# DJjjjhao/FIRA-ICSE

Hardware: AMD Instinct MI355X
Metric: training commits/sec (FIRA default config) (higher is better)
Workload: dtype f32; 1 GPU; BASELINE configs[1]: FIRA training step (fwd+bwd+Adam, dropout 0.1/0.2), batch 32 commits/GPU, fp32, 650-node graphs (mean nnz 1066/graph), vocab 24650; global_batch=32, parallelism=dp1

## Files before the change

### fira_icse_amd/csrc/engine.hip

```cpp
#include "engine.h"
#include <hip/hip_ext.h>
#include "epilogue.h"
#include <stdlib.h>
#include <map>
#include <mutex>

namespace fira {

static int64_t shadow_wbt_elems(const Layout& L);

struct Arena {
    char* base;
    size_t used = 0;
    explicit Arena(void* b) : base((char*)b) {}
    template <typename T>
    T* get(size_t n) {
        size_t bytes = (n * sizeof(T) + 255) / 256 * 256;
        T* p = base ? (T*)(base + used) : nullptr;
        used += bytes;
        return p;
    }
    float* f(size_t n) { return get<float>(n); }
};

// ... 257 lines not shown
        return gemm_bf16_ex(s, tA, tB, M, N, K, A, lda, B, ldb, C, ldc, bias, flags, splitk, colsum, c_rows, relu_mask);
    }
    return gemm_f32_ex(s, tA, tB, M, N, K, A, lda, B, ldb, C, ldc, bias, flags, splitk, colsum, c_rows, relu_mask);
}

static inline int linear(hipStream_t s, int M, int N, int K, const float* X, int ldx, const float* W, const float* b,
                         float* Y, int ldy, int flags = 0) {
    return gemm_any(s, 0, 1, M, N, K, X, ldx, W, K, Y, ldy, b, flags, 0, nullptr);
}
static inline int linear_ln(hipStream_t s, int M, int K, const float* X, int ldx, const float* W, const float* b,
                            const float* res, const float* gamma, const float* beta, float* sum, float* y, float* stats,
                            float p_drop, uint64_t seed, uint32_t st, const int32_t* y_rows = nullptr,
                            const float* r1_row = nullptr, const float* r1_col = nullptr,
                            const int32_t* slot2 = nullptr, float* y2 = nullptr, int n2 = 0, const int32_t* rows2 = nullptr,
                            uint32_t idx0 = 0) {
    bool fused = false;
    int rc = 0;
    if (g_dtype != 0 && idx0 == 0 && g_lanes == 1) {
        const uint16_t* wb;
        int ldw;
        fused = shadow_of(W, false, &wb, &ldw) && ldw == K &&
                linear_ln_bf16_try(s, M, K, X, ldx, wb, ldw, b, res, gamma, beta, sum, y, stats, p_drop, seed, st, y_rows, r1_row,
                                   r1_col, &rc);
    }
    if (fused) {
        TRY(rc);
        if (y2 && n2 > 0) TRY(rows_move(s, 0, n2, FIRA_D, y2, y, rows2, nullptr));
        return 0;
    }
    TRY(linear(s, M, FIRA_D, K, X, ldx, W, b, sum, FIRA_D));
    return add_layernorm_fwd(s, M, sum, res, gamma, beta, y, stats, p_drop, seed, st, y_rows, r1_row, r1_col, slot2, y2, idx0);
}
static inline bool linear_presum(hipStream_t s, int M, int K, const float* X, int ldx, const float* W, const float* b,
                                 const float* res, float* sum, float p_drop, uint64_t seed, uint32_t st, int* rc,
                                 uint32_t idx0 = 0) {
    if (g_dtype != 0 || !gemm_tile32_takes(1, M, FIRA_D, K, X, ldx, W, K)) return false;
    EpiRes er;
    er.res = res; er.ldr = FIRA_D; er.p = p_drop; er.inv_keep = p_drop > 0.f ? 1.0f / (1.0f - p_drop) : 1.0f;
    er.seed = seed; er.site = st; er.idx0 = idx0;
    ProfScope prof(s, PROF_GEMM, 2.0 * M * FIRA_D * (double)K, 4.0 * ((double)M * K + (double)FIRA_D * K + 2.0 * M * FIRA_D));
    return gemm_tile32_try(s, 1, M, FIRA_D, K, X, ldx, W, K, sum, FIRA_D, b, 0, rc, nullptr, nullptr, nullptr, &er);
}
static inline int linear_dgrad(hipStream_t s, int M, int N, int K, const float* dY, int lddy, const float* W, float* dX,
                               int lddx, bool accum) {
    return gemm_any(s, 0, 0, M, K, N, dY, lddy, W, K, dX, lddx, nullptr, accum ? FIRA_GEMM_ACCUM : 0, 0, nullptr);
}
struct SideStream {
    hipStream_t stream = nullptr;
    hipStream_t aux = nullptr;
    hipStream_t lane = nullptr;
    std::vector<hipEvent_t> events;
    size_t next = 0;
    bool enabled = true;
    int init() {
        if (stream) return 0;
        const char* off = getenv("FIRA_NO_WGRAD_OVERLAP");
        enabled = !(off && off[0] == '1');
        int least = 0, greatest = 0;
        if (hipDeviceGetStreamPriorityRange(&least, &greatest) != hipSuccess) least = greatest = 0;
        hipError_t e = hipStreamCreateWithPriority(&stream, hipStreamNonBlocking, least);
        if (e != hipSuccess) return set_err("hipStreamCreate: %s", hipGetErrorString(e));
        gemm_set_pad_stream(stream);
        e = hipStreamCreateWithPriority(&aux, hipStreamNonBlocking, greatest);
        if (e != hipSuccess) return set_err("hipStreamCreateWithPriority: %s", hipGetErrorString(e));
        events.resize(512);
        for (auto& ev : events) {
            e = hipEventCreateWithFlags(&ev, hipEventDisableTiming);
            if (e != hipSuccess) return set_err("hipEventCreate: %s", hipGetErrorString(e));
        }
        return 0;
    }
    hipEvent_t ev() { hipEvent_t e = events[next]; next = (next + 1) % events.size(); return e; }
};
static SideStream& side() { static thread_local SideStream s; return s; }

static int side_fork(hipStream_t main_s) {
    SideStream& sd = side();
    hipEvent_t e = sd.ev();
    if (hipEventRecord(e, main_s) != hipSuccess || hipStreamWaitEvent(sd.stream, e, 0) != hipSuccess)
        return set_err("side stream fork failed");
    return 0;
}
struct WaitProbe {
    bool on = false, init = false;
    struct Rec { int line; hipEvent_t a, b; };
    std::vector<Rec> recs;
    std::vector<hipEvent_t> pool;
    int calls = 0;
    bool enabled() {
        if (!init) { const char* e = getenv("FIRA_WAIT_PROBE"); on = e && e[0] == '1'; init = true; }
        return on;
    }
    hipEvent_t ev() {
        if (!pool.empty()) { hipEvent_t e = pool.back(); pool.pop_back(); return e; }
        hipEvent_t e = nullptr;
        (void)hipEventCreate(&e);
        return e;
    }
    void report() {
        (void)hipDeviceSynchronize();
        std::vector<std::pair<int, std::pair<double, int>>> acc;
        for (auto& r : recs) {
            float ms = 0.f;
            if (hipEventElapsedTime(&ms, r.a, r.b) != hipSuccess) ms = 0.f;
            bool found = false;
            for (auto& q : acc) if (q.first == r.line) { q.second.first += ms; q.second.second++; found = true; }
            if (!found) acc.push_back({r.line, {ms, 1}});
            pool.push_back(r.a); pool.push_back(r.b);
        }
        recs.clear();
// ... 186 lines not shown
static inline void note_graph_density(const fira_batch* b) {
    g_dense_graphs = b->n_nodes > 0 && (double)b->nnz > GCN_FUSED_MAX_DEG * (double)b->n_nodes;
}


enum Site { SITE_GATE = 0, SITE_COMB_OUT = 1, SITE_GCN = 2, SITE_SELF = 3, SITE_CROSS = 4, SITE_FFN = 5 };
static inline uint32_t site(int layer, int kind) { return (uint32_t)(layer * 8 + kind + 1); }

struct ClipStep {
    const fira_adam_opts* adam;
    float max_norm;
    fira_clip_state* state;
    void* scratch;
};
struct Ctx {
    hipStream_t s;
    const Layout* L;
    const fira_batch* bt;
    const float* P;
    float* G;
    Plan* pl;
    float p_drop, p_gcn;
    uint64_t seed;
    int R = 0;
    const int32_t* rows = nullptr;
    int Td = 0;
    const int32_t* dec_off = nullptr;
    const int32_t* row_bt = nullptr;
    const int32_t* rows_dense = nullptr;
    bool deferred = false;
    bool kv_ragged = false;
    bool serial = false;
    float* loss_sum = nullptr;
    int32_t* n_tok = nullptr;
    hipEvent_t ev_kv[16] = {};
    int kv_waited = 0;
    hipEvent_t ev_src = nullptr;
    hipEvent_t ev_zero = nullptr;
    const fira_adam_opts* adam = nullptr;
    float* Pw = nullptr;
    bool dp_begin = false;
    bool wout_planes = false;
    bool kv_planes = false;
    int32_t* row_step = nullptr;
    fira_adam_opts rows_ad{};
    bool adam_a_only = false;
    hipEvent_t ev_early = nullptr;
    const float* count = nullptr;
    const ClipStep* clip = nullptr;
    const ShadowTable* shadow_tab = nullptr;
    hipEvent_t ev_shadow = nullptr;
    int n_lanes = 1;
    struct Lane { hipStream_t s; int b0, nb, r0, nr; } lanes[2] = {};
};
typedef Ctx::Lane Lane;

static AdamRowsTables adam_rows_tables(const Layout& L, float* params, const fira_adam_opts& ad, int32_t* row_step) {
    AdamRowsTables tb;
    tb.p = params; tb.m = ad.m; tb.v = ad.v;
    tb.off[0] = L.dec_emb; tb.off[1] = L.emb;
    tb.rows[0] = tb.rows[1] = L.d.vocab;
    tb.last = row_step;
    return tb;
}

static int decoder_lanes(Ctx& c) {
    constexpr int DEC_LANES_MIN_ROWS = 768;
    static const int forced = [] { const char* e = getenv("FIRA_DEC_LANES"); return e ? (atoi(e) >= 2 ? 2 : 1) : 0; }();
    const int want = forced ? forced : (c.Td >= DEC_LANES_MIN_ROWS ? 2 : 1);
    c.n_lanes = g_lanes = 1;
    c.lanes[0] = Lane{c.s, 0, c.pl->B, 0, c.Td};
    const fira_batch& bt = *c.bt;
    if (want < 2 || !c.dec_off || !bt.dec_off_host || bt.B < 2 || !side_on() || c.serial || !c.kv_ragged) return 0;
    SideStream& sd = side();
    if (!sd.lane) {
        if (hipStreamCreateWithFlags(&sd.lane, hipStreamNonBlocking) != hipSuccess) return set_err("lane stream: create failed");
    }
    int bm = 1, best = 1 << 30;
    for (int b = 1; b < bt.B; ++b) {
        const int d = abs(2 * bt.dec_off_host[b] - c.Td);
        if (d < best) { best = d; bm = b; }
    }
    const int rm = bt.dec_off_host[bm];
    if (rm <= 0 || rm >= c.Td || bt.dec_off_host[bt.B] != c.Td) return 0;
    c.n_lanes = g_lanes = 2;
    c.lanes[0] = Lane{c.s, 0, bm, 0, rm};
    c.lanes[1] = Lane{sd.lane, bm, bt.B - bm, rm, c.Td - rm};
    return 0;
}
static int lanes_fork(Ctx& c) {
    for (int k = 1; k < c.n_lanes; ++k) {
        hipEvent_t e = side().ev();
        if (hipEventRecord(e, c.s) != hipSuccess || hipStreamWaitEvent(c.lanes[k].s, e, 0) != hipSuccess) return set_err("lane fork failed");
    }
    return 0;
}
static int lanes_join(Ctx& c) {
    for (int k = 1; k < c.n_lanes; ++k) {
        hipEvent_t e = side().ev();
        if (hipEventRecord(e, c.lanes[k].s) != hipSuccess || hipStreamWaitEvent(c.s, e, 0) != hipSuccess) return set_err("lane join failed");
    }
    return 0;
}
static int lanes_fork_to(Ctx& c, hipStream_t target) {
    for (int k = 0; k < c.n_lanes; ++k) {
        hipEvent_t e = side().ev();
        if (hipEventRecord(e, c.lanes[k].s) != hipSuccess || hipStreamWaitEvent(target, e, 0) != hipSuccess) return set_err("lane -> side stream fork failed");
    }
    return 0;
}

static inline bool fold_one_launch(int nl) { return nl <= 10; }
static inline bool comb_x3_on(int nl) { return nl <= 8; }
static inline bool gcn_x3_on(int nl) { return gcn_fused_on() && fold_one_launch(nl); }
static inline bool kv_x3_on(int nl) { return nl * 2 <= 24; }

static int adam_rows_prefetch(Ctx& c, hipStream_t st) {
    const fira_batch& bt = *c.bt;
    const Plan& p = *c.pl;
    const fira_adam_opts& ad = c.rows_ad;
    AdamRowsLists ls{};
    auto add = [&](const int32_t* ids, int n, int table) {
        if (!ids || n <= 0) return;
        const int k = ls.n_lists++;
        ls.ids[k] = ids; ls.table[k] = table;
        ls.end[k] = (k ? ls.end[k - 1] : 0) + n;
    };
    add(bt.tar, p.B * p.T, 0);
    return adam_rows_catchup(st, adam_rows_tables(*c.L, const_cast<float*>(c.P), ad, c.row_step), &ls, ad.lr, ad.beta1, ad.beta2, ad.eps,
                             ad.step - 1);
}

static int encoder_forward(Ctx& c, bool defer_memory_proj) {
    Plan& p = *c.pl;
    const Layout& L = *c.L;
    const fira_batch& bt = *c.bt;
    hipStream_t s = c.s;
    const int D = FIRA_D, Nc = bt.n_nodes, Cc = bt.n_code, Mc = bt.n_mem, KV = p.nl * 2 * D;
    hipEvent_t ev_fold0 = nullptr, ev_fold = nullptr, ev_comb = nullptr;
    bool fold_waited = false;
    {
        const bool ax = side_on() && !c.serial;
        hipStream_t fs = ax ? side().aux : s;
        if (ax) TRY(aux_fork(s));
        TransposeTable tt;
        for (int l = 0; l < p.nl && tt.n + 3 <= 24; ++l) {
            const EncLayer& w = L.enc[l];
            float* dst = p.WcT + (size_t)l * 3 * D * D;
            tt.src[tt.n] = c.P + w.wqk; tt.dst[tt.n++] = dst;
            tt.src[tt.n] = c.P + w.wqk + (size_t)D * D; tt.dst[tt.n++] = dst + (size_t)D * D;
            tt.src[tt.n] = c.P + w.wo; tt.dst[tt.n++] = dst + (size_t)2 * D * D;
        }
        TRY(transpose256_table(fs, tt));
        if (comb_x3_on(p.nl)) {
            const float* src[48];
            uint16_t* dst[48];
            int n = 0;
            for (int l = 0; l < p.nl; ++l) {
                const EncLayer& w = L.enc[l];
                const float* st[3] = {c.P + w.wqk, c.P + w.wqk + (size_t)D * D, c.P + w.wo};
                for (int j = 0; j < 3; ++j) {
                    src[n] = st[j]; dst[n++] = p.WcX + ((size_t)l * 3 + j) * 3 * D * D;
                    if (c.G) { src[n] = p.WcT + ((size_t)l * 3 + j) * D * D; dst[n++] = p.WcTX + ((size_t)l * 3 + j) * 3 * D * D; }
                }
            }
            TRY(gcn_split_planes(fs, n, src, dst));
        }
        const bool fold_one = fold_one_launch(p.nl);
        if (ax && !(fold_one && (!g_Wb || gcn_fused_on()))) TRY(side_mark(&ev_comb));
        if (fold_one) {
            const float *fW2[16], *fW1[16], *fb1[16];
            for (int l = 0; l < p.nl; ++l) { fW2[l] = c.P + L.enc[l].fc2w; fW1[l] = c.P + L.enc[l].fc1w; fb1[l] = c.P + L.enc[l].fc1b; }
            TRY(gcn_fold_weights(fs, p.nl, fW2, fW1, fb1, p.W21, gcn_fused_on() ? p.W21t : nullptr, p.c21));
            if (gcn_x3_on(p.nl)) {
                const float* src[24];
                uint16_t* dst[24];
                int n = 0;
                for (int l = 0; l < p.nl; ++l) {
                    src[n] = p.W21 + (size_t)l * D * D; dst[n++] = p.W21x + (size_t)l * 3 * D * D;
                    if (c.G) { src[n] = p.W21t + (size_t)l * D * D; dst[n++] = p.W21tx + (size_t)l * 3 * D * D; }
                }
                TRY(gcn_split_planes(fs, n, src, dst));
            }
            if (ax && (!g_Wb || gcn_fused_on())) TRY(side_mark(&ev_fold0));
        } else
        for (int l = 0; l < p.nl; ++l) {
            const EncLayer& w = L.enc[l];
            TRY(gemm_f32_ex(fs, 0, 0, D, D, D, c.P + w.fc2w, D, c.P + w.fc1w, D, p.W21 + (size_t)l * D * D, D, nullptr, 0, 0, nullptr));
            TRY(gemm_f32_ex(fs, 0, 1, D, 1, D, c.P + w.fc2w, D, c.P + w.fc1b, D, p.c21 + (size_t)l * D, 1, nullptr, 0, 0, nullptr));
            if (l == 0 && gcn_fused_on()) TRY(transpose256(fs, 1, p.W21, p.W21t));
            if (ax && l == 0 && !g_Wb && p.nl > 1) TRY(side_mark(&ev_fold0));
        }
        if (g_Wb) {
            ShadowTable t21;
            for (int l = 0; l < p.nl && l < SHADOW_MAX; ++l) {
                t21.e[l] = ShadowEntry{(int64_t)l * D * D, D, D, D, (int64_t)l * D * D};
                t21.tile_start[l + 1] = t21.tile_start[l] + cdiv(D, 64) * cdiv(D, 64);
                t21.n = l + 1;
            }
            TRY(weight_shadows(fs, t21, p.W21, p.w21b, p.w21bt));
            g_W21 = p.W21; g_W21n = (int64_t)p.nl * D * D; g_W21b = p.w21b; g_W21bT = p.w21bt;
        }
        if (!fold_one && gcn_fused_on() && p.nl > 1) TRY(transpose256(fs, p.nl - 1, p.W21 + (size_t)D * D, p.W21t + (size_t)D * D));
        if (ax && !(ev_fold0 && fold_one && gcn_fused_on())) TRY(side_mark(&ev_fold));
        if (!ev_fold0) ev_fold0 = ev_fold;
        if (c.shadow_tab) {
            TRY(weight_shadows(fs, *c.shadow_tab, c.P, p.wb, p.wbt));
            if (ax) TRY(side_mark(&c.ev_shadow));
        }
    }
    const int32_t* head_list = c.dec_off ? c.rows_dense : c.rows;
    TRY(prep(s, p.B, p.L, p.S, p.T, bt.sou, bt.sub_token, bt.tar, p.mem_valid, bt.tar ? p.tar_valid : nullptr, p.pos_code,
             p.pos_tar, c.R, head_list, bt.tar ? p.compact_row : nullptr, head_list ? nullptr : p.iota, c.loss_sum, c.n_tok,
             Nc, bt.code_rows, Cc, p.code_slot, bt.mem_rows, Mc, p.mem_slot, c.dec_off, p.row_bt, p.rows_c, bt.mem_dst,
             p.mem_off, p.mem_valid_c));
    c.kv_ragged = true;
    AdamRowsView vw_emb;
    if (c.row_step)
        vw_emb = adam_rows_view(adam_rows_tables(L, nullptr, c.rows_ad, c.row_step), 1, c.rows_ad.lr, c.rows_ad.beta1, c.rows_ad.beta2,
                                c.rows_ad.eps, c.rows_ad.step - 1);
    TRY(node_features(s, Nc, bt.node_rows, p.N, p.L, p.S, bt.sou, bt.sub_token, bt.ast_change, c.P + L.emb, c.P + L.ast_emb,
                      p.pos_code, p.X[0], p.code_slot, p.enc[0].Xc, &vw_emb));
    TRY(linear(s, 4, p.nl * D, D, c.P + L.mark_emb, D, c.P + L.w2_all, c.P + L.b2_all, p.vtab_all, p.nl * D));
    for (int l = 0; l < p.nl; ++l) {
        const EncLayer& w = L.enc[l];
        EncSave& e = p.enc[l];
        float* X = p.X[l];
        if (l < 8) {
            if (l == 0 && ev_comb) TRY(main_wait(s, ev_comb, __LINE__));
            else if (l == 0 && ev_fold0) { TRY(main_wait(s, ev_fold0, __LINE__)); fold_waited = true; }
            const float* wt = p.WcT + (size_t)l * 3 * D * D;
            TRY(comb_fused_fwd(s, Cc, e.Xc, wt, wt + (size_t)D * D, wt + (size_t)2 * D * D, c.P + w.bqk, c.P + w.bo,
                               p.vtab_all + l * D, p.nl * D, bt.code_mark, e.qk, e.c, c.P + w.ln1g, c.P + w.ln1b, e.s1, X,
                               bt.code_rows, e.st1, c.p_drop, c.seed, site(l, SITE_GATE), site(l, SITE_COMB_OUT), g_dtype == 1,
                               comb_x3_on(p.nl) ? p.WcX + (size_t)l * 9 * D * D : nullptr));
        } else {
        TRY(linear(s, Cc, 2 * D, D, e.Xc, D, c.P + w.wqk, c.P + w.bqk, e.qk, 2 * D));
        TRY(combination_fwd(s, Cc, e.qk, p.vtab_all + l * D, p.nl * D, bt.code_mark, e.c, c.p_drop, c.seed, site(l, SITE_GATE)));
        TRY(linear_ln(s, Cc, D, e.c, D, c.P + w.wo, c.P + w.bo, e.Xc, c.P + w.ln1g, c.P + w.ln1b, e.s1, X, e.st1, c.p_drop,
                      c.seed, site(l, SITE_COMB_OUT), bt.code_rows));
        }
        const bool fused = gcn_fused_on();
        if (!fused) TRY(csr_spmm_ex(s, Nc, bt.rowptr, bt.col, bt.val, X, D, e.Z, D, 0, 1, 0, l == 0 ? p.rsum : nullptr));
        if (l == 0 && ev_fold0 && !fold_waited) TRY(main_wait(s, ev_fold0, __LINE__));
        if (l == 1 && ev_fold && ev_fold != ev_fold0) TRY(main_wait(s, ev_fold, __LINE__));
        const bool last = l + 1 == p.nl;
        if (fused)
            TRY(gcn_fused_fwd(s, Nc, bt.rowptr, bt.col, bt.val, X, p.W21t + (size_t)l * D * D, c.P + w.fc2b, p.c21 + (size_t)l * D,
                              c.P + w.ln2g, c.P + w.ln2b, e.s2, p.X[l + 1], e.st2, l == 0 ? p.rsum : nullptr,
                              last ? p.mem_slot : p.code_slot, last ? p.mem_c : p.enc[l + 1].Xc, c.p_gcn, c.seed,
                              site(l, SITE_GCN), g_dtype == 1, gcn_x3_on(p.nl) ? p.W21x + (size_t)l * 3 * D * D : nullptr));
        else
        TRY(linear_ln(s, Nc, D, e.Z, D, p.W21 + (size_t)l * D * D, c.P + w.fc2b, X, c.P + w.ln2g, c.P + w.ln2b, e.s2,
                      p.X[l + 1], e.st2, c.p_gcn, c.seed, site(l, SITE_GCN), nullptr, p.rsum, p.c21 + (size_t)l * D,
                      last ? p.mem_slot : p.code_slot, last ? p.mem_c : p.enc[l + 1].Xc, last ? Mc : Cc,
                      last ? bt.mem_rows : bt.code_rows));
    }
    c.deferred = false;
    if (defer_memory_proj && side_on() && p.nl <= 16) {
        TRY(aux_fork(s));
        hipStream_t ss = side().aux;
        const bool kvx = c.G && kv_x3_on(p.nl);
        if (kvx) {
            const float* src[24];
            uint16_t* dst[24];
            for (int j = 0; j < p.nl * 2; ++j) { src[j] = c.P + L.wkv_all + (size_t)j * D * D; dst[j] = p.WkvX + (size_t)j * 3 * D * D; }
            TRY(gcn_split_planes(ss, p.nl * 2, src, dst));
        }
        for (int l = 0; l < p.nl; ++l) {
            const size_t o = (size_t)l * 2 * D;
            if (kvx) {
                const int l1 = l == 0 ? std::min(2, p.nl) : p.nl;
                if (l == 0 || l == std::min(2, p.nl))
                    TRY(linear_x3(ss, Mc, p.mem_c, D, p.WkvX + (size_t)l * 2 * 3 * D * D, (l1 - l) * 2, c.P + L.bkv_all + o, p.kv_all + o,
                                  p.kvp, g_dtype == 1));
            } else
            TRY(gemm_any(ss, 0, 1, Mc, 2 * D, D, p.mem_c, D, c.P + L.wkv_all + o * D, D, p.kv_all + o, p.kvp, c.P + L.bkv_all + o, 0,
                         0, nullptr));
            if (l == std::min(1, p.nl - 1) || l == p.nl - 1) TRY(side_mark(&c.ev_kv[l]));
        }
        TRY(gemm_any(ss, 0, 1, Mc, D, D, p.mem_c, D, c.P + L.ws, D, p.src, D, nullptr, 0, 0, nullptr, bt.mem_dst));
        TRY(side_mark(&c.ev_src));
        if (kvx && p.nl * 2 <= 24) {
            TransposeTable tt;
            const float* src[24];
            uint16_t* dst[24];
            for (int j = 0; j < p.nl * 2; ++j) {
                tt.src[tt.n] = c.P + L.wkv_all + (size_t)j * D * D; tt.dst[tt.n++] = p.WkvT + (size_t)j * D * D;
                src[j] = p.WkvT + (size_t)j * D * D; dst[j] = p.WkvTX + (size_t)j * 3 * D * D;
            }
            TRY(transpose256_table(ss, tt));
            TRY(gcn_split_planes(ss, p.nl * 2, src, dst));
            c.kv_planes = true;
        }
        if (c.G && g_dtype == 1) {
            TRY(split_planes_t(ss, c.P + L.wout, p.V, p.WoutTX, true));
            c.wout_planes = true;
        }
        c.deferred = true;
        return 0;
    }
    TRY(gemm_any(s, 0, 1, Mc, KV, D, p.mem_c, D, c.P + L.wkv_all, D, p.kv_all, p.kvp, c.P + L.bkv_all, 0, 0, nullptr));
    TRY(gemm_any(s, 0, 1, Mc, D, D, p.mem_c, D, c.P + L.ws, D, p.src, D, nullptr, 0, 0, nullptr, bt.mem_dst));
    return 0;
}

static int decoder_forward(Ctx& c) {
    Plan& p = *c.pl;
    const Layout& L = *c.L;
    const int D = FIRA_D, H = L.d.n_head, Sm = p.L + p.S;
    if (c.row_bt) {
        AdamRowsView vw;
        if (c.row_step)
            vw = adam_rows_view(adam_rows_tables(L, nullptr, c.rows_ad, c.row_step), 0, c.rows_ad.lr, c.rows_ad.beta1, c.rows_ad.beta2,
                                c.rows_ad.eps, c.rows_ad.step - 1);
        TRY(embed_rows_fwd(c.s, c.Td, p.T, c.row_bt, c.bt->tar, c.P + L.dec_emb, p.pos_tar, p.x0, &vw));
    } else {
        if (c.row_step) TRY(adam_rows_prefetch(c, c.s));
        TRY(embed_gather_fwd(c.s, p.B, p.T, c.bt->tar, c.P + L.dec_emb, p.pos_tar, p.x0, p.T, 0));
    }
    ProfDecoderTag prof_tag;
    TRY(decoder_lanes(c));
    ProfScope prof_region(c.s, PROF_DEC_REGION, 0.0);
    TRY(lanes_fork(c));
    struct LaneState {
        const float *x = nullptr, *pend_sum = nullptr, *pend_g = nullptr, *pend_b = nullptr;
        float *pend_y = nullptr, *pend_st = nullptr;
        int kv_waited = 0;
    } state[2];
    for (int k = 0; k < c.n_lanes; ++k) state[k].x = p.x0;
    for (int l = 0; l < p.nl; ++l) {
        const DecLayer& w = L.dec[l];
        DecSave& e = p.dec[l];
        const bool last = l + 1 == p.nl;
        for (int k = 0; k < c.n_lanes; ++k) {
            const Lane& ln = c.lanes[k];
            LaneState& st = state[k];
            hipStream_t s = ln.s;
            const size_t r0 = (size_t)ln.r0;
            const int nr = ln.nr;
            const uint32_t idx0 = (uint32_t)(r0 * D);
            auto consume = [&](int N, const float* W, const float* b, float* Y, int flags) -> int {
                if (st.pend_sum) {
                    int rc = 0;
                    float* sum = const_cast<float*>(st.pend_sum) + r0 * D;
                    const bool fused = gemm_tile32_ln_try(s, nr, N, sum, D, W, b, Y + r0 * N, N, flags, st.pend_g, st.pend_b,
                                                          st.pend_y + r0 * D, st.pend_st + r0 * 2, &rc);
                    if (!fused)
                        rc = add_layernorm_fwd(s, nr, sum, nullptr, st.pend_g, st.pend_b, st.pend_y + r0 * D, st.pend_st + r0 * 2, 0.f, 0, 0,
                                               nullptr);
                    st.pend_sum = nullptr;
                    if (rc || fused) return rc;
                }
                return linear(s, nr, N, D, st.x + r0 * D, D, W, b, Y + r0 * N, N, flags);
            };
            auto close_block = [&](int K, const float* X, const float* W, const float* b, const float* res, const float* g,
                                   const float* be, float* sum, float* y, float* stt, uint32_t site_id, bool may_defer,
                                   const int32_t* slot2, float* y2, int n2, const int32_t* rows2) -> int {
                int rc = 0;
                if (may_defer && linear_presum(s, nr, K, X + r0 * K, K, W, b, res + r0 * D, sum + r0 * D, c.p_drop, c.seed, site_id,
                                               &rc, idx0)) {
                    st.pend_sum = sum; st.pend_g = g; st.pend_b = be; st.pend_y = y; st.pend_st = stt;
                    return rc;
                }
                return linear_ln(s, nr, K, X + r0 * K, K, W, b, res + r0 * D, g, be, sum + r0 * D, y + r0 * D, stt + r0 * 2, c.p_drop,
                                 c.seed, site_id, nullptr, nullptr, nullptr, slot2 ? slot2 + r0 : nullptr, y2, n2, rows2, idx0);
            };
            const int32_t* q_off = c.dec_off ? c.dec_off + ln.b0 : nullptr;
            TRY(consume(3 * D, c.P + w.wqkv, c.P + w.bqkv, e.qkv, 0));
            TRY(attention_fwd(s, ln.nb, H, p.T, p.T, e.qkv, 3 * D, e.qkv + D, 3 * D, e.qkv + 2 * D, 3 * D, p.tar_valid + (size_t)ln.b0 * p.T,
                              1, 0, e.ao, D, q_off, 1, attn_bf16()));
            TRY(close_block(D, e.ao, c.P + w.wo_s, c.P + w.bo_s, st.x, c.P + w.lns_g, c.P + w.lns_b, e.s_a, e.x_a, e.st_a,
                            site(l, SITE_SELF), true, nullptr, nullptr, 0, nullptr));
            st.x = e.x_a;
            TRY(consume(D, c.P + w.wq_c, c.P + w.bq_c, e.qc, 0));
            if (c.deferred) {
                int m = l;
                while (m < p.nl - 1 && c.ev_kv[m] == nullptr) ++m;
                if (c.ev_kv[m] != nullptr && st.kv_waited < m + 1) {
                    TRY(main_wait(s, c.ev_kv[m], __LINE__));
                    st.kv_waited = m + 1;
                }
            }
            TRY(attention_fwd(s, ln.nb, H, p.T, Sm, e.qc, D, p.kv_all + l * 2 * D, p.kvp, p.kv_all + l * 2 * D + D, p.kvp,
                              c.kv_ragged ? p.mem_valid_c : p.mem_valid, 0, 0, e.ao2, D, q_off, 0, attn_bf16(),
                              c.kv_ragged ? p.mem_off + ln.b0 : nullptr));
            TRY(close_block(D, e.ao2, c.P + w.wo_c, c.P + w.bo_c, e.x_a, c.P + w.lnc_g, c.P + w.lnc_b, e.s_c, e.x_c, e.st_c,
                            site(l, SITE_CROSS), true, nullptr, nullptr, 0, nullptr));
            st.x = e.x_c;
            TRY(consume(p.F, c.P + w.w1, c.P + w.b1, e.h, FIRA_GEMM_RELU));
            const bool head_copy = last && c.rows != nullptr && c.R > 0;
            TRY(close_block(p.F, e.h, c.P + w.w2, c.P + w.b2, e.x_c, c.P + w.lnf_g, c.P + w.lnf_b, e.s_f, e.x_f, e.st_f,
                            site(l, SITE_FFN), !last, head_copy ? p.compact_row : nullptr, head_copy ? p.dec_c : nullptr,
                            head_copy ? c.R : 0, head_copy ? c.rows : nullptr));
            st.x = e.x_f;
        }
    }
    TRY(lanes_join(c));
    return 0;
}

static int head_forward(Ctx& c, int R, const int32_t* rows, float* loss_sum, int32_t* n_tok, int32_t* argmax_out,
                        int want_grad) {
    Plan& p = *c.pl;
    const Layout& L = *c.L;
    hipStream_t s = c.s;
    const int D = FIRA_D, Sm = p.L + p.S;
    const float* dec = p.dec[p.nl - 1].x_f;
    const float* dec_rows = (c.rows != nullptr && rows == c.rows) ? p.dec_c : dec;
    if (dec_rows == dec && R != c.Td) {
        TRY(rows_gather_idx(s, R, p.dec_c, dec, rows));
        dec_rows = p.dec_c;
    }
    if (g_dtype == 0 && R >= 64 && R <= p.TB)
        TRY(head_logits_x3(s, R, p.V, dec_rows, D, c.P + L.wout, c.P + L.bout, p.logits, p.ldl, p.xh_planes));
    else
    TRY(linear(s, R, p.V, D, dec_rows, D, c.P + L.wout, c.P + L.bout, p.logits, p.ldl));
    TRY(gemm_any(s, 0, 1, c.Td, D, D, dec, D, c.P + L.wt, D, p.tgt, D, nullptr, 0, 0, nullptr));
    if (c.deferred) TRY(main_wait(s, c.ev_src, __LINE__));
    TRY(copy_score_fwd_ex(s, p.B, p.T, Sm, p.src, p.tgt, c.P + L.wres, c.P + L.bres, p.score, 1, p.mem_valid,
                          argmax_out ? nullptr : c.bt->tar_label, p.V, c.dec_off));
    TRY(linear(s, c.Td, 2, D, dec, D, c.P + L.wp, c.P + L.bp, p.gate, 2));
    TRY(head_loss(s, c.Td, p.T, p.V, Sm, p.compact_row, p.logits, p.ldl, p.score, p.mem_valid, p.gate,
                  c.bt->tar_label, loss_sum, n_tok, argmax_out, want_grad, c.row_bt));
    return 0;
}

static inline int enc_wgrad_every(int n_rows, int n_layers) {
    static const int forced = [] { const char* e = getenv("FIRA_ENC_WGRAD_EVERY"); const int v = e ? atoi(e) : 0; return v >= 1 ? v : 0; }();
    if (forced) return forced;
    return n_rows <= 32768 ? std::max(1, n_layers) : 1;
}

static int group_a_final_stream(hipStream_t s, hipStream_t* out) {
    SideStream& sd = side();
    *out = s;
    if (sd.stream && sd.enabled) {
        TRY(aux_fork(s));
        hipEvent_t e2 = sd.ev();
        if (hipEventRecord(e2, sd.stream) != hipSuccess || hipStreamWaitEvent(sd.aux, e2, 0) != hipSuccess)
            return set_err("group-A mark: weight-gradient stream mark failed");
        *out = sd.aux;
    }
    return 0;
}

struct BwdMid {
    hipEvent_t ev_dmem = nullptr;
    hipEvent_t ev_groupA = nullptr;
};

static int backward_decoder(Ctx& c, int R, const int32_t* rows, hipEvent_t mid_event, BwdMid& mid) {
    Plan& p = *c.pl;
    const Layout& L = *c.L;
    hipStream_t s = c.s;
    const int D = FIRA_D, H = L.d.n_head, KV = p.nl * 2 * D, Sm = p.L + p.S;
    const fira_batch& bt = *c.bt;
    const int Nc = bt.n_nodes, Cc = bt.n_code, Mc = bt.n_mem;
    const float* dec = p.dec[p.nl - 1].x_f;
    float* G = c.G;

    gemm_group_reset();
    gemm_bf16_group_reset();
    gemm_wgrad_panel_reset();
    gemm_wgrad_panel_scratch(p.panel_scratch, p.panel_floats);
    red().reset(p.red_buf, p.red_cap);
    const bool so = side_on();
    hipStream_t ss = so ? side().aux : s;
    hipEvent_t ev_dfc = nullptr;
    if (c.ev_zero) TRY(main_wait(s, c.ev_zero, __LINE__));
    else TRY(zero(s, p.zero_beg, (size_t)((char*)p.zero_end - (char*)p.zero_beg)));
    if (R > 0) {
        if (so) TRY(aux_fork(s));
        if (c.wout_planes) TRY(dgrad_x3_splitk(ss, R, p.V, p.logits, p.ldl, p.WoutTX, p.ddec_c, D, g_dtype == 1));
        else
// ... 431 lines not shown
                      int32_t* n_tok, void* mid_event, float* params_w, const fira_adam_opts* adam, bool begin_only = false,
                      int32_t* row_step = nullptr, const ClipStep* clip = nullptr) {
    const Layout* L = get_layout(d);
    if (!L) return 1;
    TRY(check_batch(batch));
    FIRA_REQUIRE(batch->tar && batch->tar_label, "training batch needs tar and tar_label");
    FIRA_REQUIRE(params && grads && workspace && loss_sum && n_tok, "null pointer argument");
    Plan p;
    const size_t need = p.build(workspace, *d, batch->B, true);
    FIRA_REQUIRE(need <= workspace_bytes, "workspace too small: need %zu bytes, got %zu", need, workspace_bytes);
    TRY(check_counts(batch, p));
    Ctx c{(hipStream_t)stream, L, batch, params, grads, &p, opts ? opts->dropout : 0.f, opts ? opts->gcn_dropout : 0.f,
          opts ? opts->seed : 0};
    FIRA_REQUIRE(c.p_drop >= 0.f && c.p_drop < 1.f && c.p_gcn >= 0.f && c.p_gcn < 1.f, "dropout must be in [0,1)");
    FIRA_REQUIRE(!opts || opts->dtype == 0 || opts->dtype == 1, "fira_train_opts.dtype must be 0 (fp32) or 1 (bf16)");
    DtypeScope dtype_scope(opts ? opts->dtype : 0);
    TRY(side().init());
    const bool bf16 = opts && opts->dtype == 1;
    const ShadowTable* tab = bf16 ? shadow_table(*L) : nullptr;
    ShadowScope shadow_scope(params, L->total, bf16 ? p.wb : nullptr, bf16 ? p.wbt : nullptr, tab);
    const bool defer_sh = bf16 && side_on() && gcn_fused_on() && L->d.n_layer <= 8;
    if (bf16 && !defer_sh) TRY(weight_shadows(c.s, *tab, params, p.wb, p.wbt));
    if (defer_sh) c.shadow_tab = tab;
    c.Td = p.TB;
    if (opts && opts->compact_dec && batch->dec_off) {
        FIRA_REQUIRE(batch->n_dec_rows >= batch->B && batch->n_dec_rows <= p.TB, "bad n_dec_rows %d", batch->n_dec_rows);
        c.Td = batch->n_dec_rows;
        c.dec_off = batch->dec_off;
        c.row_bt = p.row_bt;
    }
    int R = c.Td;
    const int32_t* rows = p.iota;
    if (opts && opts->compact_head && batch->head_rows) {
        R = batch->n_head_rows;
        FIRA_REQUIRE(R >= 0 && R <= c.Td, "bad n_head_rows %d", R);
        c.rows_dense = batch->head_rows;
        rows = c.dec_off ? p.rows_c : batch->head_rows;
        c.R = R;
        c.rows = rows;
    }
    c.loss_sum = loss_sum;
    c.n_tok = n_tok;
    c.adam = adam;
    c.Pw = params_w;
    const bool zero_g = opts && opts->zero_grads;
    if (!side_on() && zero_g) TRY(zero(c.s, grads, (size_t)L->live * sizeof(float)));
    if (adam && row_step && L->d.d_model == FIRA_D) {
        c.row_step = row_step;
        c.rows_ad = *adam;
    }
    c.dp_begin = begin_only;
    if (begin_only) c.adam = nullptr;
    if (clip) { c.adam = nullptr; c.clip = clip; }
    TRY(encoder_forward(c, true));
    if (side_on()) {
        TRY(zero(side().aux, p.zero_beg, (size_t)((char*)p.zero_end - (char*)p.zero_beg)));
        TRY(zero(side().aux, p.dXa, (size_t)batch->n_nodes * FIRA_D * sizeof(float)));
        if (zero_g) TRY(zero(side().aux, grads, (size_t)L->live * sizeof(float)));
        TRY(side_mark(&c.ev_zero));
    }
    if (c.ev_shadow) TRY(main_wait(c.s, c.ev_shadow, __LINE__));
    TRY(decoder_forward(c));
    TRY(head_forward(c, R, rows, loss_sum, n_tok, nullptr, 1));
    if (begin_only) {
        PendingStep& ps = g_pending;
        ps.active = false;
        ps.mid = BwdMid();
        TRY(backward_decoder(c, R, rows, (hipEvent_t)mid_event, ps.mid));
        ps.plan = p;
        ps.batch = *batch;
        ps.ctx = c;
        ps.ctx.pl = &ps.plan;
        ps.ctx.bt = &ps.batch;
        ps.dtype = opts ? opts->dtype : 0;
        ps.params = params;
        ps.tab = tab;
        ps.W21 = g_W21; ps.W21n = g_W21n; ps.W21b = g_W21b; ps.W21bT = g_W21bT;
        ps.active = true;
        return 0;
    }
    TRY(backward(c, R, rows, (hipEvent_t)mid_event));
    if (wait_probe().enabled() && ++wait_probe().calls == 20) wait_probe().report();
    return 0;
}

int fira_train_fwd_bwd(void* stream, const fira_dims* d, const fira_batch* batch, const float* params, float* grads,
                       void* workspace, size_t workspace_bytes, const fira_train_opts* opts, float* loss_sum,
                       int32_t* n_tok, void* mid_event) {
    return train_call(stream, d, batch, params, grads, workspace, workspace_bytes, opts, loss_sum, n_tok, mid_event, nullptr,
                      nullptr);
}

int fira_ffn_fwd(void* stream, int M, int F, const float* x, const float* w1, const float* b1, const float* w2, const float* b2,
                 const float* gamma, const float* beta, float* h, float* sum, float* y, float* stats, float dropout,
                 uint64_t seed, uint32_t site_id, int dtype) {
    FIRA_REQUIRE(x && w1 && b1 && w2 && b2 && gamma && beta && h && sum && y && stats && M > 0 && F > 0, "fira_ffn_fwd: bad argument");
    FIRA_REQUIRE(dropout >= 0.f && dropout < 1.f && (dtype == 0 || dtype == 1), "fira_ffn_fwd: bad dropout / dtype");
    DtypeScope dtype_scope(dtype);
    hipStream_t s = (hipStream_t)stream;
    const int D = FIRA_D;
    TRY(linear(s, M, F, D, x, D, w1, b1, h, F, FIRA_GEMM_RELU));
    return linear_ln(s, M, F, h, F, w2, b2, x, gamma, beta, sum, y, stats, dropout, seed, site_id);
}
int fira_ffn_bwd(void* stream, int M, int F, const float* dy, const float* x, const float* h, const float* sum,
                 const float* stats, const float* w1, const float* w2, const float* gamma, float* dx, float* dyf_ws,
                 float* dh_ws, float* dw1, float* db1, float* dw2, float* db2, float* dgamma, float* dbeta, float dropout,
// ... 424 lines not shown
```

Before: 14110 commits/s.

## Overlap decoder layer-0 self-attention and copy-score head with encoder on aux stream

Splits the decoder layer into self-attention and rest parts so that the embedding and layer-0 self-attention (which do not depend on the encoder) can be issued on the aux stream during the encoder forward. The main stream then waits on an event before the cross-attention. In the head, the copy-score path (tgt GEMM, copy score, gate) moves to the aux stream concurrently with the vocab logits GEMM. This exposes more concurrency in a latency-bound step, at the cost of extra events and cross-stream ordering that must respect dropout seeds and the zeroing done on the aux stream. The behaviour is on by default and can be disabled with FIRA_SERIAL_CHAIN=1.

Result: slower. 13850 commits/s (-1.8%).

```diff
diff --git a/fira_icse_amd/csrc/engine.hip b/fira_icse_amd/csrc/engine.hip
--- a/fira_icse_amd/csrc/engine.hip
+++ b/fira_icse_amd/csrc/engine.hip
@@ -333,10 +333,13 @@
     std::vector<hipEvent_t> events;
     size_t next = 0;
     bool enabled = true;
+    bool serial_chain = false;
     int init() {
         if (stream) return 0;
         const char* off = getenv("FIRA_NO_WGRAD_OVERLAP");
         enabled = !(off && off[0] == '1');
+        const char* ser = getenv("FIRA_SERIAL_CHAIN");
+        serial_chain = ser && ser[0] == '1';
         int least = 0, greatest = 0;
         if (hipDeviceGetStreamPriorityRange(&least, &greatest) != hipSuccess) least = greatest = 0;
         hipError_t e = hipStreamCreateWithPriority(&stream, hipStreamNonBlocking, least);
@@ -629,6 +632,10 @@
     hipEvent_t ev_shadow = nullptr;
     int n_lanes = 1;
     struct Lane { hipStream_t s; int b0, nb, r0, nr; } lanes[2] = {};
+    bool chain_overlap = false;
+    hipEvent_t ev_self0 = nullptr;
+    const float *self0_pend_sum = nullptr, *self0_pend_g = nullptr, *self0_pend_b = nullptr;
+    float *self0_pend_y = nullptr, *self0_pend_st = nullptr;
 };
 typedef Ctx::Lane Lane;
 
@@ -707,6 +714,8 @@
     return adam_rows_catchup(st, adam_rows_tables(*c.L, const_cast<float*>(c.P), ad, c.row_step), &ls, ad.lr, ad.beta1, ad.beta2, ad.eps,
                              ad.step - 1);
 }
+
+static int decoder_self0_early(Ctx& c);
 
 static int encoder_forward(Ctx& c, bool defer_memory_proj) {
     Plan& p = *c.pl;
@@ -792,6 +801,7 @@
              Nc, bt.code_rows, Cc, p.code_slot, bt.mem_rows, Mc, p.mem_slot, c.dec_off, p.row_bt, p.rows_c, bt.mem_dst,
              p.mem_off, p.mem_valid_c));
     c.kv_ragged = true;
+    TRY(decoder_self0_early(c));
     AdamRowsView vw_emb;
     if (c.row_step)
         vw_emb = adam_rows_view(adam_rows_tables(L, nullptr, c.rows_ad, c.row_step), 1, c.rows_ad.lr, c.rows_ad.beta1, c.rows_ad.beta2,
@@ -882,97 +892,136 @@
     return 0;
 }
 
-static int decoder_forward(Ctx& c) {
+struct DecLaneState {
+    const float *x = nullptr, *pend_sum = nullptr, *pend_g = nullptr, *pend_b = nullptr;
+    float *pend_y = nullptr, *pend_st = nullptr;
+    int kv_waited = 0;
+};
+static int decoder_embed(Ctx& c, hipStream_t s) {
     Plan& p = *c.pl;
     const Layout& L = *c.L;
-    const int D = FIRA_D, H = L.d.n_head, Sm = p.L + p.S;
     if (c.row_bt) {
         AdamRowsView vw;
         if (c.row_step)
             vw = adam_rows_view(adam_rows_tables(L, nullptr, c.rows_ad, c.row_step), 0, c.rows_ad.lr, c.rows_ad.beta1, c.rows_ad.beta2,
                                 c.rows_ad.eps, c.rows_ad.step - 1);
-        TRY(embed_rows_fwd(c.s, c.Td, p.T, c.row_bt, c.bt->tar, c.P + L.dec_emb, p.pos_tar, p.x0, &vw));
-    } else {
-        if (c.row_step) TRY(adam_rows_prefetch(c, c.s));
-        TRY(embed_gather_fwd(c.s, p.B, p.T, c.bt->tar, c.P + L.dec_emb, p.pos_tar, p.x0, p.T, 0));
-    }
+        return embed_rows_fwd(s, c.Td, p.T, c.row_bt, c.bt->tar, c.P + L.dec_emb, p.pos_tar, p.x0, &vw);
+    }
+    if (c.row_step) TRY(adam_rows_prefetch(c, s));
+    return embed_gather_fwd(s, p.B, p.T, c.bt->tar, c.P + L.dec_emb, p.pos_tar, p.x0, p.T, 0);
+}
+enum { DEC_SELF = 1, DEC_REST = 2 };
+static int decoder_layer_fwd(Ctx& c, int l, int k, DecLaneState& st, hipStream_t s, int parts) {
+    Plan& p = *c.pl;
+    const Layout& L = *c.L;
+    const int D = FIRA_D, H = L.d.n_head, Sm = p.L + p.S;
+    const DecLayer& w = L.dec[l];
+    DecSave& e = p.dec[l];
+    const bool last = l + 1 == p.nl;
+    const Lane& ln = c.lanes[k];
+    const size_t r0 = (size_t)ln.r0;
+    const int nr = ln.nr;
+    const uint32_t idx0 = (uint32_t)(r0 * D);
+    auto consume = [&](int N, const float* W, const float* b, float* Y, int flags) -> int {
+        if (st.pend_sum) {
+            int rc = 0;
+            float* sum = const_cast<float*>(st.pend_sum) + r0 * D;
+            const bool fused = gemm_tile32_ln_try(s, nr, N, sum, D, W, b, Y + r0 * N, N, flags, st.pend_g, st.pend_b,
+                                                  st.pend_y + r0 * D, st.pend_st + r0 * 2, &rc);
+            if (!fused)
+                rc = add_layernorm_fwd(s, nr, sum, nullptr, st.pend_g, st.pend_b, st.pend_y + r0 * D, st.pend_st + r0 * 2, 0.f, 0, 0,
+                                       nullptr);
+            st.pend_sum = nullptr;
+            if (rc || fused) return rc;
+        }
+        return linear(s, nr, N, D, st.x + r0 * D, D, W, b, Y + r0 * N, N, flags);
+    };
+    auto close_block = [&](int K, const float* X, const float* W, const float* b, const float* res, const float* g,
+                           const float* be, float* sum, float* y, float* stt, uint32_t site_id, bool may_defer,
+                           const int32_t* slot2, float* y2, int n2, const int32_t* rows2) -> int {
+        int rc = 0;
+        if (may_defer && linear_presum(s, nr, K, X + r0 * K, K, W, b, res + r0 * D, sum + r0 * D, c.p_drop, c.seed, site_id,
+                                       &rc, idx0)) {
+            st.pend_sum = sum; st.pend_g = g; st.pend_b = be; st.pend_y = y; st.pend_st = stt;
+            return rc;
+        }
+        return linear_ln(s, nr, K, X + r0 * K, K, W, b, res + r0 * D, g, be, sum + r0 * D, y + r0 * D, stt + r0 * 2, c.p_drop,
+                         c.seed, site_id, nullptr, nullptr, nullptr, slot2 ? slot2 + r0 : nullptr, y2, n2, rows2, idx0);
+    };
+    const int32_t* q_off = c.dec_off ? c.dec_off + ln.b0 : nullptr;
+    if (parts & DEC_SELF) {
+        TRY(consume(3 * D, c.P + w.wqkv, c.P + w.bqkv, e.qkv, 0));
+        TRY(attention_fwd(s, ln.nb, H, p.T, p.T, e.qkv, 3 * D, e.qkv + D, 3 * D, e.qkv + 2 * D, 3 * D, p.tar_valid + (size_t)ln.b0 * p.T,
+                          1, 0, e.ao, D, q_off, 1, attn_bf16()));
+        TRY(close_block(D, e.ao, c.P + w.wo_s, c.P + w.bo_s, st.x, c.P + w.lns_g, c.P + w.lns_b, e.s_a, e.x_a, e.st_a,
+                        site(l, SITE_SELF), true, nullptr, nullptr, 0, nullptr));
+        st.x = e.x_a;
+    }
+    if (!(parts & DEC_REST)) return 0;
+    TRY(consume(D, c.P + w.wq_c, c.P + w.bq_c, e.qc, 0));
+    if (c.deferred) {
+        int m = l;
+        while (m < p.nl - 1 && c.ev_kv[m] == nullptr) ++m;
+        if (c.ev_kv[m] != nullptr && st.kv_waited < m + 1) {
+            TRY(main_wait(s, c.ev_kv[m], __LINE__));
+            st.kv_waited = m + 1;
+        }
+    }
+    TRY(attention_fwd(s, ln.nb, H, p.T, Sm, e.qc, D, p.kv_all + l * 2 * D, p.kvp, p.kv_all + l * 2 * D + D, p.kvp,
+                      c.kv_ragged ? p.mem_valid_c : p.mem_valid, 0, 0, e.ao2, D, q_off, 0, attn_bf16(),
+                      c.kv_ragged ? p.mem_off + ln.b0 : nullptr));
+    TRY(close_block(D, e.ao2, c.P + w.wo_c, c.P + w.bo_c, e.x_a, c.P + w.lnc_g, c.P + w.lnc_b, e.s_c, e.x_c, e.st_c,
+                    site(l, SITE_CROSS), true, nullptr, nullptr, 0, nullptr));
+    st.x = e.x_c;
+    TRY(consume(p.F, c.P + w.w1, c.P + w.b1, e.h, FIRA_GEMM_RELU));
+    const bool head_copy = last && c.rows != nullptr && c.R > 0;
+    TRY(close_block(p.F, e.h, c.P + w.w2, c.P + w.b2, e.x_c, c.P + w.lnf_g, c.P + w.lnf_b, e.s_f, e.x_f, e.st_f,
+                    site(l, SITE_FFN), !last, head_copy ? p.compact_row : nullptr, head_copy ? p.dec_c : nullptr,
+                    head_copy ? c.R : 0, head_copy ? c.rows : nullptr));
+    st.x = e.x_f;
+    return 0;
+}
+
+static int decoder_self0_early(Ctx& c) {
+    c.ev_self0 = nullptr;
+    if (!c.chain_overlap || !side_on() || c.serial || c.pl->nl < 1) return 0;
+    const int lanes_before = g_lanes;
+    TRY(decoder_lanes(c));
+    if (c.n_lanes != 1) { g_lanes = lanes_before; return 0; }
+    ProfDecoderTag prof_tag;
+    TRY(aux_fork(c.s));
+    hipStream_t as = side().aux;
+    TRY(decoder_embed(c, as));
+    DecLaneState st;
+    st.x = c.pl->x0;
+    TRY(decoder_layer_fwd(c, 0, 0, st, as, DEC_SELF));
+    TRY(side_mark(&c.ev_self0));
+    c.self0_pend_sum = st.pend_sum; c.self0_pend_g = st.pend_g; c.self0_pend_b = st.pend_b;
+    c.self0_pend_y = st.pend_y; c.self0_pend_st = st.pend_st;
+    g_lanes = lanes_before;
+    return 0;
+}
+
+static int decoder_forward(Ctx& c) {
+    Plan& p = *c.pl;
+    const bool early = c.ev_self0 != nullptr;
+    if (!early) TRY(decoder_embed(c, c.s));
     ProfDecoderTag prof_tag;
     TRY(decoder_lanes(c));
     ProfScope prof_region(c.s, PROF_DEC_REGION, 0.0);
     TRY(lanes_fork(c));
-    struct LaneState {
-        const float *x = nullptr, *pend_sum = nullptr, *pend_g = nullptr, *pend_b = nullptr;
-        float *pend_y = nullptr, *pend_st = nullptr;
-        int kv_waited = 0;
-    } state[2];
+    DecLaneState state[2];
     for (int k = 0; k < c.n_lanes; ++k) state[k].x = p.x0;
-    for (int l = 0; l < p.nl; ++l) {
-        const DecLayer& w = L.dec[l];
-        DecSave& e = p.dec[l];
-        const bool last = l + 1 == p.nl;
-        for (int k = 0; k < c.n_lanes; ++k) {
-            const Lane& ln = c.lanes[k];
-            LaneState& st = state[k];
-            hipStream_t s = ln.s;
-            const size_t r0 = (size_t)ln.r0;
-            const int nr = ln.nr;
-            const uint32_t idx0 = (uint32_t)(r0 * D);
-            auto consume = [&](int N, const float* W, const float* b, float* Y, int flags) -> int {
-                if (st.pend_sum) {
-                    int rc = 0;
-                    float* sum = const_cast<float*>(st.pend_sum) + r0 * D;
-                    const bool fused = gemm_tile32_ln_try(s, nr, N, sum, D, W, b, Y + r0 * N, N, flags, st.pend_g, st.pend_b,
-                                                          st.pend_y + r0 * D, st.pend_st + r0 * 2, &rc);
-                    if (!fused)
-                        rc = add_layernorm_fwd(s, nr, sum, nullptr, st.pend_g, st.pend_b, st.pend_y + r0 * D, st.pend_st + r0 * 2, 0.f, 0, 0,
-                                               nullptr);
-                    st.pend_sum = nullptr;
-                    if (rc || fused) return rc;
-                }
-                return linear(s, nr, N, D, st.x + r0 * D, D, W, b, Y + r0 * N, N, flags);
-            };
-            auto close_block = [&](int K, const float* X, const float* W, const float* b, const float* res, const float* g,
-                                   const float* be, float* sum, float* y, float* stt, uint32_t site_id, bool may_defer,
-                                   const int32_t* slot2, float* y2, int n2, const int32_t* rows2) -> int {
-                int rc = 0;
-                if (may_defer && linear_presum(s, nr, K, X + r0 * K, K, W, b, res + r0 * D, sum + r0 * D, c.p_drop, c.seed, site_id,
-                                               &rc, idx0)) {
-                    st.pend_sum = sum; st.pend_g = g; st.pend_b = be; st.pend_y = y; st.pend_st = stt;
-                    return rc;
-                }
-                return linear_ln(s, nr, K, X + r0 * K, K, W, b, res + r0 * D, g, be, sum + r0 * D, y + r0 * D, stt + r0 * 2, c.p_drop,
-                                 c.seed, site_id, nullptr, nullptr, nullptr, slot2 ? slot2 + r0 : nullptr, y2, n2, rows2, idx0);
-            };
-            const int32_t* q_off = c.dec_off ? c.dec_off + ln.b0 : nullptr;
-            TRY(consume(3 * D, c.P + w.wqkv, c.P + w.bqkv, e.qkv, 0));
-            TRY(attention_fwd(s, ln.nb, H, p.T, p.T, e.qkv, 3 * D, e.qkv + D, 3 * D, e.qkv + 2 * D, 3 * D, p.tar_valid + (size_t)ln.b0 * p.T,
-                              1, 0, e.ao, D, q_off, 1, attn_bf16()));
-            TRY(close_block(D, e.ao, c.P + w.wo_s, c.P + w.bo_s, st.x, c.P + w.lns_g, c.P + w.lns_b, e.s_a, e.x_a, e.st_a,
-                            site(l, SITE_SELF), true, nullptr, nullptr, 0, nullptr));
-            st.x = e.x_a;
-            TRY(consume(D, c.P + w.wq_c, c.P + w.bq_c, e.qc, 0));
-            if (c.deferred) {
-                int m = l;
-                while (m < p.nl - 1 && c.ev_kv[m] == nullptr) ++m;
-                if (c.ev_kv[m] != nullptr && st.kv_waited < m + 1) {
-                    TRY(main_wait(s, c.ev_kv[m], __LINE__));
-                    st.kv_waited = m + 1;
-                }
-            }
-            TRY(attention_fwd(s, ln.nb, H, p.T, Sm, e.qc, D, p.kv_all + l * 2 * D, p.kvp, p.kv_all + l * 2 * D + D, p.kvp,
-                              c.kv_ragged ? p.mem_valid_c : p.mem_valid, 0, 0, e.ao2, D, q_off, 0, attn_bf16(),
-                              c.kv_ragged ? p.mem_off + ln.b0 : nullptr));
-            TRY(close_block(D, e.ao2, c.P + w.wo_c, c.P + w.bo_c, e.x_a, c.P + w.lnc_g, c.P + w.lnc_b, e.s_c, e.x_c, e.st_c,
-                            site(l, SITE_CROSS), true, nullptr, nullptr, 0, nullptr));
-            st.x = e.x_c;
-            TRY(consume(p.F, c.P + w.w1, c.P + w.b1, e.h, FIRA_GEMM_RELU));
-            const bool head_copy = last && c.rows != nullptr && c.R > 0;
-            TRY(close_block(p.F, e.h, c.P + w.w2, c.P + w.b2, e.x_c, c.P + w.lnf_g, c.P + w.lnf_b, e.s_f, e.x_f, e.st_f,
-                            site(l, SITE_FFN), !last, head_copy ? p.compact_row : nullptr, head_copy ? p.dec_c : nullptr,
-                            head_copy ? c.R : 0, head_copy ? c.rows : nullptr));
-            st.x = e.x_f;
-        }
-    }
+    if (early) {
+        DecLaneState& st = state[0];
+        st.x = p.dec[0].x_a;
+        st.pend_sum = c.self0_pend_sum; st.pend_g = c.self0_pend_g; st.pend_b = c.self0_pend_b;
+        st.pend_y = c.self0_pend_y; st.pend_st = c.self0_pend_st;
+        TRY(main_wait(c.s, c.ev_self0, __LINE__));
+    }
+    for (int l = 0; l < p.nl; ++l)
+        for (int k = 0; k < c.n_lanes; ++k)
+            TRY(decoder_layer_fwd(c, l, k, state[k], c.lanes[k].s, l == 0 && early ? DEC_REST : DEC_SELF | DEC_REST));
     TRY(lanes_join(c));
     return 0;
 }
@@ -989,15 +1038,23 @@
         TRY(rows_gather_idx(s, R, p.dec_c, dec, rows));
         dec_rows = p.dec_c;
     }
+    const bool ov = c.chain_overlap && side_on() && !c.serial;
+    hipStream_t cs = ov ? side().aux : s;
+    hipEvent_t ev_copy = nullptr;
+    if (ov) TRY(aux_fork(s));
     if (g_dtype == 0 && R >= 64 && R <= p.TB)
         TRY(head_logits_x3(s, R, p.V, dec_rows, D, c.P + L.wout, c.P + L.bout, p.logits, p.ldl, p.xh_planes));
     else
     TRY(linear(s, R, p.V, D, dec_rows, D, c.P + L.wout, c.P + L.bout, p.logits, p.ldl));
-    TRY(gemm_any(s, 0, 1, c.Td, D, D, dec, D, c.P + L.wt, D, p.tgt, D, nullptr, 0, 0, nullptr));
-    if (c.deferred) TRY(main_wait(s, c.ev_src, __LINE__));
-    TRY(copy_score_fwd_ex(s, p.B, p.T, Sm, p.src, p.tgt, c.P + L.wres, c.P + L.bres, p.score, 1, p.mem_valid,
+    TRY(gemm_any(cs, 0, 1, c.Td, D, D, dec, D, c.P + L.wt, D, p.tgt, D, nullptr, 0, 0, nullptr));
+    if (c.deferred && !ov) TRY(main_wait(s, c.ev_src, __LINE__));
+    TRY(copy_score_fwd_ex(cs, p.B, p.T, Sm, p.src, p.tgt, c.P + L.wres, c.P + L.bres, p.score, 1, p.mem_valid,
                           argmax_out ? nullptr : c.bt->tar_label, p.V, c.dec_off));
-    TRY(linear(s, c.Td, 2, D, dec, D, c.P + L.wp, c.P + L.bp, p.gate, 2));
+    TRY(linear(cs, c.Td, 2, D, dec, D, c.P + L.wp, c.P + L.bp, p.gate, 2));
+    if (ov) {
+        TRY(side_mark(&ev_copy));
+        TRY(main_wait(s, ev_copy, __LINE__));
+    }
     TRY(head_loss(s, c.Td, p.T, p.V, Sm, p.compact_row, p.logits, p.ldl, p.score, p.mem_valid, p.gate,
                   c.bt->tar_label, loss_sum, n_tok, argmax_out, want_grad, c.row_bt));
     return 0;
@@ -1535,6 +1592,7 @@
     c.dp_begin = begin_only;
     if (begin_only) c.adam = nullptr;
     if (clip) { c.adam = nullptr; c.clip = clip; }
+    c.chain_overlap = side_on() && !side().serial_chain;
     TRY(encoder_forward(c, true));
     if (side_on()) {
         TRY(zero(side().aux, p.zero_beg, (size_t)((char*)p.zero_end - (char*)p.zero_beg)));
```
